# SamuelCancilla2/radar-point-cloud-tracking

Measured on AMD Instinct MI355X. Metric: Mpoints/s clustered+tracked, 1024-echo synthetic frames; 1/2/4/8-GPU scaling, higher is better.
Workload: dtype u8 echo / f32 geometry / f64 distance

## Files before the change

### radar-point-cloud-tracking_amd/csrc/stdbscan.hip

```cpp
#include <algorithm>
#include <cfloat>
#include <climits>
#include <cmath>
#include <cstdlib>
#include <cstring>
#include <mutex>
#include <type_traits>
#include <vector>

#include "common.h"
#include "dispatch.h"

#pragma clang fp contract(off)

namespace rpt {

namespace {

#include "stdbscan_shared.inc"
#include "stdbscan_grid.inc"
#include "stdbscan_core.inc"
#include "stdbscan_union.inc"
#include "stdbscan_label.inc"
#include "stdbscan_frames.inc"
// ... 17 lines not shown
  }
  double ms(int i) {
    float t = 0;
    (void)hipEventElapsedTime(&t, ev[i], ev[i + 1]);
    return t;
  }
  ~Timer() {
    for (auto& e : ev)
      if (e) (void)hipEventDestroy(e);
  }
};

}

struct DbscanState {
  Scratch arena;
  int dim = 2;
  int64_t n = 0;
  bool degenerate = false;
  int32_t min_samples = 0;
  Geom g{};
  int64_t C = 0, nt = 0;
  float4* pts = nullptr;
  int32_t *sorig = nullptr, *skey = nullptr, *cell_start = nullptr, *rep = nullptr;
  uint8_t *mutual = nullptr, *core = nullptr;
  float2* slab_t = nullptr;
  int32_t *parent = nullptr, *ccmin = nullptr, *cid = nullptr, *nc_list = nullptr;
  int32_t *occ = nullptr, *hpos = nullptr;
  const int32_t* n_occ_dev = nullptr;
  uint64_t* cell_min_pair = nullptr;
  bool cmin_ready = false;
  void* crec = nullptr;
  uint32_t* occ_bits = nullptr;
  uint4* pmask = nullptr;
  int union_cpw() const {
    if (ab().union_cpw) return ab().union_cpw;
    return n > (int64_t(1) << 24) ? 64 : 16;
  }
  uint32_t* min_bits = nullptr;
  int32_t* min_pref = nullptr;
  int64_t min_words() const { return n / 32 + 1; }
  int32_t* n_clusters_ptr() const { return min_pref + min_words(); }
  int32_t cluster_ids(hipStream_t st, int32_t* cell_key, int32_t* zero = nullptr);
  int32_t* cell_root = nullptr;
  bool bucket_allmin = false;
  bool k5_fused_path() const {
    return oct_ok() && ab().k5_mode == 0 && ab().k5_fused && !ab().k5_tiles;
  }
  int32_t* rowq = nullptr;
  int32_t* rowcnt = nullptr;
  bool rowq_ok = false;
  int tile_by = 0, tile_nbands = 0, tile_R = 0;
  bool use_label_tiles() const { return ab().k7_tiles && rowq_ok && dim == 2 && g.nz == 1; }
  unsigned tile_grid_blocks() const {
    return (unsigned)((((int64_t)g.nt * tile_nbands + 1) + 7) & ~(int64_t)7);
  }
  double slab_reach() const {
    return integral_t ? std::ceil(std::floor((double)g.epst) / g.ct)
                      : std::ceil((double)g.epst / g.ct) + 1.0;
  }
  bool oct_ok() const { return dim == 2 && g.nz == 1 && slab_reach() <= (double)kCwMaxR; }
  template <int D>
  const CellRec<D>* rec() const {
    return static_cast<const CellRec<D>*>(crec);
  }
  int32_t* slab = nullptr;
  bool spos_on = false;
  bool dense_slabs = false;
  int32_t* cell_min = nullptr;
  uint8_t* fok = nullptr;
  bool integral_t = false;
  bool all_mutual = false;
  bool cell_comp = false;
  bool cell_comp_ok() const {
    const AbSwitches& a = ab();
    return all_mutual && dim == 2 && a.union_list && a.union_pair && a.union_nm && a.cell_comp &&
           !use_label_tiles() && !a.uf_compress;
  }
  bool xy_points = false;
  bool may_xy = false;
  bool xy_rule() const {
    const AbSwitches& a = ab();
    return a.xy_points && dim == 2 && g.tfree && g.epst == std::floor(g.epst) && cell_comp_ok() &&
           k5_fused_path() && (int)slab_reach() <= 2 && a.k5_mask && !a.k7_tiles && a.k7_w == 32;
  }
  int32_t need_float4(const char* who) const {
    if (!xy_points) return RPT_OK;
    set_error("%s: internal: this state's sorted points are xy-only", who);
    return RPT_EHIP;
  }
  template <bool XY>
  Pt<XY>* points() const {
    return reinterpret_cast<Pt<XY>*>(pts);
  }
  int64_t* stmp = nullptr;
  Timer tm;

  template <int D>
  int32_t build_t(const float* x, const float* y, const float* z, int64_t stride, const float* t,
                  double eps_space, double eps_time, hipStream_t st);
  const void* given_bounds = nullptr;
  int32_t build(const float* x, const float* y, const float* z, int64_t stride, const float* t,
                int64_t n_, double eps_space, double eps_time, int32_t ms, bool timing,
                hipStream_t st);
  int32_t core_pass(hipStream_t st);
  int32_t union_pass(hipStream_t st, bool fused = false);
  int32_t labels_local(int32_t* labels, rpt_stdbscan_stats* stats, hipStream_t st);
  bool defer = false;
  int32_t fill_stats(int32_t n_clusters, rpt_stdbscan_stats* stats);
  int32_t labels_global(const int64_t* rep_orig, const int64_t* reps, int64_t nr,
                        int32_t* labels, hipStream_t st, const int64_t* nr_dev = nullptr);
// ... 90 lines not shown
    g.tfree = (g.rt >= 0 && ct == 1.0 && (double)g.rt <= std::floor((double)epst)) ? 1 : 0;
  }
  all_mutual = D == 2 && integral_t && ct == 1.0 && hb.n_finite_t == n && min_samples >= 1 &&
               epst >= 0.f && eps_space > 0.0 && 2.0 * cs * cs <= g.eps2 * (1.0 - 1e-6);
  C = g.cells;
  const int64_t C1 = C + 1;
  Budget bud;
  bud.add<Bounds>(1);
  for (int k = 0; k < 4; ++k) bud.add<uint32_t>(n);
  bud.add<int64_t>(radix_tmp_elems(n));
  bud.add<float4>(n);
  bud.add<int32_t>(n);
  bud.add<int32_t>(n);
  bud.add<int32_t>(C1 + 1);
  bud.add<int64_t>(scan_tmp_elems(C1 + 1) + scan_tmp_elems(n + 1));
  bud.add<uint8_t>(C1);
  bud.add<int32_t>(C1);
  bud.add<float2>(nt);
  bud.add<uint8_t>(n);
  bud.add<int32_t>(n);
  bud.add<int32_t>(n);
  bud.add<int32_t>(n + 1);
  bud.add<int32_t>(n + 1);
  bud.add<int32_t>(n);
  bud.add<uint8_t>(C1);
  bud.add<int32_t>(C1);
  bud.add<int32_t>(C1);
  bud.add<uint64_t>(C1);
  bud.add<uint32_t>(n / 32 + 1);
  bud.add<int32_t>(n / 32 + 2);
  bud.add<int32_t>(n + 1);
  bud.add<int32_t>(n + 1);
  bud.add<CellRec<D>>(C1);
  bud.add<uint32_t>(C1 / 32 + 2);
  bud.add<int32_t>(nt + 1);
  bud.add<int32_t>(nt + 1);
  bud.add<int32_t>(nt + 1);
  bud.add<int32_t>((size_t)(ny * nz * nt) + 1);
  bud.add<int32_t>((size_t)(ny * nz * nt) + 1);
  RPT_TRY(arena.reserve(bud.bytes, st));
  (void)arena.carve_n<Bounds>(1);
  uint32_t* keys = arena.carve_n<uint32_t>(n);
  uint32_t* vals = arena.carve_n<uint32_t>(n);
  uint32_t* keys_alt = arena.carve_n<uint32_t>(n);
  uint32_t* vals_alt = arena.carve_n<uint32_t>(n);
  pmask = reinterpret_cast<uint4*>(keys);
  int64_t* rtmp = arena.carve_n<int64_t>(radix_tmp_elems(n));
  pts = arena.carve_n<float4>(n);
  sorig = arena.carve_n<int32_t>(n);
  skey = arena.carve_n<int32_t>(n);
  cell_start = arena.carve_n<int32_t>(C1 + 1);
  stmp = arena.carve_n<int64_t>(scan_tmp_elems(C1 + 1) + scan_tmp_elems(n + 1));
  mutual = arena.carve_n<uint8_t>(C1);
  rep = arena.carve_n<int32_t>(C1);
  slab_t = arena.carve_n<float2>(nt);
  core = arena.carve_n<uint8_t>(n);
  parent = arena.carve_n<int32_t>(n);
  ccmin = arena.carve_n<int32_t>(n);
  cid = arena.carve_n<int32_t>(n + 1);
  nc_list = arena.carve_n<int32_t>(n + 1);
  slab = arena.carve_n<int32_t>(n);
  fok = arena.carve_n<uint8_t>(C1);
  cell_min = arena.carve_n<int32_t>(C1);
  cell_root = arena.carve_n<int32_t>(C1);
  cell_min_pair = arena.carve_n<uint64_t>(C1);
  min_bits = arena.carve_n<uint32_t>(n / 32 + 1);
  min_pref = arena.carve_n<int32_t>(n / 32 + 2);
  occ = arena.carve_n<int32_t>(n + 1);
  hpos = arena.carve_n<int32_t>(n + 1);
  CellRec<D>* cr = arena.carve_n<CellRec<D>>(C1);
  crec = cr;
  occ_bits = arena.carve_n<uint32_t>(C1 / 32 + 2);
  int32_t* slab_lo = arena.carve_n<int32_t>(nt + 1);
  int32_t* slab_occ = arena.carve_n<int32_t>(nt + 1);
  int32_t* occ_base = arena.carve_n<int32_t>(nt + 1);
  rowq = arena.carve_n<int32_t>((size_t)(ny * nz * nt) + 1);
  rowcnt = arena.carve_n<int32_t>((size_t)(ny * nz * nt) + 1);
  rowq_ok = false;
  if (!slab_lo || !rowcnt) {
    set_error("internal: scratch carve overflow");
    return RPT_ENOMEM;
  }
  bucket_allmin = false;
  const bool bucket = ab().k4_bucket && D == 2 && hb.n_finite_t == n && !hb.t_descends &&
                      (int64_t)nx * ny <= kBucketCells && nt < (int64_t(1) << 31);
  xy_points = may_xy && bucket && D == 2 && hb.n_finite_t == n && xy_rule();
  float2* const slab_t_w = xy_points ? slab_t : nullptr;
  if (bucket) {
    hipLaunchKernelGGL(k_slab_lo, dim3(grid_for(64 * (nt + 1), kBlock, 4096)), dim3(kBlock), 0,
                       st, t, n, g, slab_lo, occ_bits, (int64_t)(C1 / 32 + 2));
    const size_t hist_bytes = sizeof(int32_t) * (size_t)nx * ny;
    const int64_t avg = n / std::max<int64_t>(nt, 1);
    dense_slabs = avg > 8 * kChunkPts;
    spos_on = ab().label_orig == 2 || (ab().label_orig == 1 && dense_slabs);
    int32_t* spos_w = spos_on ? slab : nullptr;
    int64_t ch = avg > 8 * kChunkPts ? (avg + kChunkPts - 1) / kChunkPts : 1;
    ch = std::max<int64_t>(ch, (512 + nt - 1) / std::max<int64_t>(nt, 1));
    int CH = (int)std::min<int64_t>(ch, 64);
    while (CH > 1 && (int64_t)nt * CH * nx * ny > 4 * n) --CH;
    if (ab().slab_chunks > 0) CH = ab().slab_chunks;
    const bool coalesced_scan = CH >= 8 && (int64_t)nt * CH * nx * ny <= 4 * n &&
                                !ab().chunk_scan;
    if (CH > 1 && (int64_t)nt * CH * nx * ny <= 4 * n) {
      int32_t* hist_g = reinterpret_cast<int32_t*>(keys);
      RPT_HIP(hipFuncSetAttribute((const void*)k_slab_chunk_hist,
// ... 269 lines not shown
    hipLaunchKernelGGL(k_core_slow<3>, dim3(wave_grid(n)), dim3(kBlock), 0, st, pts, skey, g,
                       rec<3>(), occ_bits, slab_t, slow, n_slow, core);
  RPT_CHECK_LAUNCH();
  cmin_ready = cm != nullptr;
  tm.mark();
  return RPT_OK;
}

int32_t DbscanState::union_pass(hipStream_t st, bool fused) {
  cell_comp = false;
  if (degenerate) return RPT_OK;
  const AbSwitches& a = ab();
  const int uf_flags = a.uf_flags;
  const int gb = grid_for(n, kBlock, 2048);
  const int gw = wave_grid(n);
  const unsigned gp = (unsigned)((n + kBlock - 1) / kBlock);
  const int32_t* n_occ = n_occ_dev;
  auto* cmin = reinterpret_cast<unsigned long long*>(cell_min_pair);
  const bool listing = a.union_list && dim == 2;
  int32_t* plist = listing ? nc_list : nullptr;
  int32_t* pcount = listing ? nc_list + n : nullptr;
  const bool nm = dim == 2 && a.union_pair && a.union_nm;
  int32_t* nm_list = nm ? cid : nullptr;
  int32_t* nm_count = nm ? cid + n : nullptr;
  cell_comp = fused && cell_comp_ok();
  if (!cell_comp) RPT_TRY(need_float4("union_pass"));
  if (!cell_comp || !cmin_ready)
    hipLaunchKernelGGL(k_init_occ_cells, dim3(gb), dim3(kBlock), 0, st, occ, n_occ, C, rep,
                       cmin_ready ? nullptr : cmin, pcount, nm_count);
  if (!cmin_ready)
    hipLaunchKernelGGL(k_cell_min_pair, dim3(gb), dim3(kBlock), 0, st, skey, core, sorig, n, C,
                       cmin);
  if (cell_comp)
    hipLaunchKernelGGL(k_parent_init_cells, dim3(gb), dim3(kBlock), 0, st, occ, n_occ, C, cmin,
                       rep, parent, pcount, nm_count, min_bits, min_words(), cell_min);
  else
    hipLaunchKernelGGL(k_parent_init_pair, dim3(grid_for(n, kBlock * kPU, 2048)), dim3(kBlock), 0,
                       st, parent, n, core, skey, mutual, cmin, C, rep);
  int32_t* lstat_dev = nullptr;
  if (dim == 2) {
    uint4* pm = listing ? pmask : nullptr;
    if (a.union_pair)
      hipLaunchKernelGGL(k_union_cells_pair, dim3(gw), dim3(kBlock), 0, st, pts, g, occ, n_occ,
                         rec<2>(), occ_bits, slab_t, rep, mutual, sorig, parent, uf_flags, pm,
                         plist, pcount, union_cpw(), nm_list, nm_count);
    else
      hipLaunchKernelGGL((k_union_cells<2, false>), dim3(gw), dim3(kBlock), 0, st, pts, g,
                         cell_start, occ, n_occ, rec<2>(), occ_bits, slab_t, core, rep, mutual,
                         sorig, parent, uf_flags, pm, plist, pcount);
#ifdef RPT_AB
    if (listing && ab().stats) {
      static int32_t* buf = nullptr;
      if (!buf) (void)hipMalloc(&buf, 16);
      lstat_dev = buf;
      (void)hipMemsetAsync(lstat_dev, 0, 16, st);
    }
#endif
    if (listing) {
      const bool snap = ab().union_snap == 2 || (ab().union_snap == 1 && !dense_slabs);
      if (snap)
        hipLaunchKernelGGL(k_cell_root_snapshot, dim3(grid_for(n, kBlock, 4096)), dim3(kBlock),
                           0, st, occ, n_occ, rep, parent, g.cells, uf_flags, cell_root);
      const int32_t* croot = snap ? (const int32_t*)cell_root : nullptr;
      with_bool(xy_points, [&](auto xy) {
        hipLaunchKernelGGL(k_union_listed<xy.value>, dim3(gw), dim3(kBlock), 0, st,
                           points<xy.value>(), g, occ, rec<2>(), occ_bits, slab_t, core, rep,
                           mutual, sorig, parent, uf_flags, pm, plist, pcount, croot, lstat_dev);
      });
    }
    else
      hipLaunchKernelGGL((k_union_cells<2, true>), dim3(gw), dim3(kBlock), 0, st, pts, g,
                         cell_start, occ, n_occ, rec<2>(), occ_bits, slab_t, core, rep, mutual,
                         sorig, parent, uf_flags, pm, plist, pcount);
    if (cell_comp) {
    } else if (nm)
      hipLaunchKernelGGL(k_union_nm<2>, dim3(gw), dim3(kBlock), 0, st, pts, g, cell_start,
                         rec<2>(), slab_t, core, rep, mutual, sorig, parent, nm_list, nm_count);
    else
// ... 42 lines not shown
                       occ, n_occ_dev, C, mutual, rep, cell_root, zero, min_bits, W, cell_key);
  } else {
    RPT_HIP(hipMemsetAsync(min_bits, 0, sizeof(uint32_t) * W, st));
    if (zero) RPT_HIP(hipMemsetAsync(zero, 0, sizeof(int32_t), st));
    if (cell_key)
      hipLaunchKernelGGL(k_fill_i32, dim3(grid_for(C, kBlock, 8192)), dim3(kBlock), 0, st,
                         cell_key, C, INT_MAX);
  }
  hipLaunchKernelGGL(k_ccmin, dim3(tile_grid(n)), dim3(kBlock), 0, st, parent, core, n, sorig,
                     ccmin, min_bits, nc_list, nc_list + n, skey, mutual,
                     cr ? (const int32_t*)cell_root : nullptr, C, cell_key);
  hipLaunchKernelGGL(k_word_popc, dim3(grid_for(W, kBlock, 2048)), dim3(kBlock), 0, st, min_bits,
                     W, min_pref);
  RPT_CHECK_LAUNCH();
  return exclusive_scan_total_i32(min_pref, min_pref, W, st);
}

int32_t DbscanState::labels_local(int32_t* labels, rpt_stdbscan_stats* stats, hipStream_t st) {
  const int gb = grid_for(n, kBlock, 2048);
  if (degenerate) {
    hipLaunchKernelGGL(k_isolated_labels, dim3(gb), dim3(kBlock), 0, st, labels, n,
                       min_samples <= 0 ? 1 : 0);
    RPT_CHECK_LAUNCH();
    if (stats) {
      stats->n_points = n;
      stats->n_core = min_samples <= 0 ? n : 0;
      stats->n_clusters = min_samples <= 0 ? (int32_t)n : 0;
    }
    return RPT_OK;
  }
  int32_t* nc_count = nc_list + n;
  const MinRank mr{min_bits, min_pref};
  const unsigned glc = (unsigned)((grid_for(n, kBlock * kPU, 2048) + 7) & ~7);
  if (cell_comp) {
    const int64_t W = min_words();
    hipLaunchKernelGGL(k_cell_comp, dim3(grid_for(n, kBlock, 2048)), dim3(kBlock), 0, st, parent,
                       occ, n_occ_dev, C, rep, sorig, cell_min, min_bits, nc_count);
    hipLaunchKernelGGL(k_word_popc, dim3(grid_for(W, kBlock, 2048)), dim3(kBlock), 0, st,
                       min_bits, W, min_pref);
    RPT_CHECK_LAUNCH();
    RPT_TRY(exclusive_scan_total_i32(min_pref, min_pref, W, st));
    with_bool(spos_on, [&](auto orig) {
      hipLaunchKernelGGL(k_label_core_cells<orig.value>, dim3(glc), dim3(kBlock), 0, st, skey,
                         core, orig.value ? slab : sorig, n, C, cell_min, mr, labels, nc_list,
                         nc_count, cid + n, n_clusters_ptr());
    });
  } else {
    RPT_TRY(cluster_ids(st, cell_min, nc_count));
    if (spos_on)
      hipLaunchKernelGGL(k_label_core_orig, dim3(glc), dim3(kBlock), 0, st, ccmin, n, slab, mr,
                         labels);
    else
      hipLaunchKernelGGL(k_label_core, dim3(glc), dim3(kBlock), 0, st, ccmin, n, sorig, mr,
                         labels);
  }
  if (!cell_comp || ab().k7_w != 32 || use_label_tiles()) RPT_TRY(need_float4("labels_local"));
  int32_t* kstat = nullptr;
#ifdef RPT_AB
  if (ab().stats) {
    static int32_t* buf = nullptr;
    if (!buf) (void)hipMalloc(&buf, 16);
    kstat = buf;
    (void)hipMemsetAsync(kstat, 0, 16, st);
  }
#endif
#ifdef RPT_AB
  if (use_label_tiles())
    hipLaunchKernelGGL((k_label_tiles<false>), dim3(tile_grid_blocks()), dim3(kTileBlock), 0, st,
                       g, tile_R, tile_by, tile_nbands, (int64_t)g.nt * tile_nbands, occ,
                       n_occ_dev, rowq, rec<2>(), mutual, occ_bits, slab_t, pts, ccmin, cell_min,
                       sorig, mr, min_samples, labels);
  else if (cell_comp && ab().k7_w == 64)
    hipLaunchKernelGGL((k_label<2, false, 64, true>), dim3(wave_grid(n)), dim3(kBlock), 0, st,
                       pts, skey, g, rec<2>(), occ_bits, slab_t, (const int32_t*)nullptr,
                       cell_min, mutual, sorig, mr, nc_list, nc_count, labels,
                       (int32_t*)nullptr, core);
  else if (dim == 2 && ab().k7_w == 64)
    hipLaunchKernelGGL((k_label<2, false, 64>), dim3(wave_grid(n)), dim3(kBlock), 0, st, pts,
                       skey, g, rec<2>(), occ_bits, slab_t, ccmin, cell_min, mutual, sorig, mr,
                       nc_list, nc_count, labels);
  else
#endif
  if (cell_comp && xy_points)
    hipLaunchKernelGGL((k_label<2, false, 32, true, true>), dim3(wave_grid(n)), dim3(kBlock), 0,
                       st, reinterpret_cast<const Pt<true>*>(pts), skey, g, rec<2>(), occ_bits,
                       slab_t, (const int32_t*)nullptr, cell_min, mutual, sorig, mr, nc_list,
                       nc_count, labels, kstat, core);
  else if (cell_comp)
    hipLaunchKernelGGL((k_label<2, false, 32, true>), dim3(wave_grid(n)), dim3(kBlock), 0, st,
                       pts, skey, g, rec<2>(), occ_bits, slab_t, (const int32_t*)nullptr,
                       cell_min, mutual, sorig, mr, nc_list, nc_count, labels, kstat, core);
  else if (dim == 2)
    hipLaunchKernelGGL((k_label<2, false, 32>),
                       dim3(wave_grid(n)), dim3(kBlock), 0, st, pts, skey, g,
                       rec<2>(), occ_bits, slab_t, ccmin, cell_min, mutual, sorig, mr, nc_list,
                       nc_count, labels, kstat);
  else
    hipLaunchKernelGGL((k_label<3, false, 64>),
                       dim3(wave_grid(n)), dim3(kBlock), 0, st, pts, skey, g,
                       rec<3>(), occ_bits, slab_t, ccmin, cell_min, mutual, sorig, mr, nc_list,
                       nc_count, labels);
  RPT_CHECK_LAUNCH();
#ifdef RPT_AB
  if (kstat) {
    int32_t ks[4] = {0, 0, 0, 0};
    (void)hipMemcpyAsync(ks, kstat, 16, hipMemcpyDeviceToHost, st);
    (void)hipStreamSynchronize(st);
    std::fprintf(stderr,
                 "[rpt stats] n=%lld label: queued=%d core_in_window=%d searched=%d labelled=%d\n",
                 (long long)n, ks[0], ks[1], ks[2], ks[3]);
  }
#endif
  tm.mark();
  if (stats && defer) return RPT_OK;
  if (stats) {
    int32_t ncl = 0;
    RPT_HIP(hipMemcpyAsync(&ncl, n_clusters_ptr(), sizeof(int32_t), hipMemcpyDeviceToHost, st));
    RPT_TRY(wait_stream(st));
    RPT_TRY(fill_stats(ncl, stats));
  }
  return RPT_OK;
}

int32_t DbscanState::fill_stats(int32_t ncl, rpt_stdbscan_stats* stats) {
// ... 447 lines not shown
```

### radar-point-cloud-tracking_amd/csrc/stdbscan_label.inc

```

__global__ __launch_bounds__(kBlock) void k_fill_i32(int32_t* p, int64_t n, int32_t v) {
  for (int64_t i = (int64_t)blockIdx.x * blockDim.x + threadIdx.x; i < n;
       i += (int64_t)gridDim.x * blockDim.x)
    p[i] = v;
}

struct MinRank {
  const uint32_t* bits;
  const int32_t* pref;
  __device__ __forceinline__ int32_t operator[](int32_t m) const {
    const uint32_t w = bits[m >> 5];
    return pref[m >> 5] + __popc(w & ((1u << (m & 31)) - 1u));
  }
};

__global__ void k_word_popc(const uint32_t* __restrict__ bits, int64_t words,
                            int32_t* __restrict__ out) {
  for (int64_t i = (int64_t)blockIdx.x * blockDim.x + threadIdx.x; i < words;
       i += (int64_t)gridDim.x * blockDim.x)
    out[i] = __popc(bits[i]);
}

__global__ __launch_bounds__(kBlock) void k_cell_roots(int32_t* parent,
                                                      const int32_t* __restrict__ occ,
// ... 177 lines not shown
#pragma unroll
    for (int u = 0; u < kPU; ++u) {
      const int64_t i = tile + (int64_t)u * kBlock + threadIdx.x;
      if (i < n && own[u] >= 0)
        labels[i] = pr[u] + __popc(w[u] & ((1u << (own[u] & 31)) - 1u));
    }
  }
}

__global__ __launch_bounds__(kBlock) void k_cell_comp(int32_t* parent,
                                                     const int32_t* __restrict__ occ,
                                                     const int32_t* __restrict__ n_occ,
                                                     int64_t cells,
                                                     const int32_t* __restrict__ rep,
                                                     const int32_t* __restrict__ sorig,
                                                     int32_t* __restrict__ cell_key,
                                                     uint32_t* __restrict__ min_bits,
                                                     int32_t* __restrict__ zero) {
  if (blockIdx.x == 0 && threadIdx.x == 0) *zero = 0;
  const int64_t m = *n_occ;
  for (int64_t q = (int64_t)blockIdx.x * blockDim.x + threadIdx.x; q < m;
       q += (int64_t)gridDim.x * blockDim.x) {
    const int32_t c = occ[q];
    if ((int64_t)c >= cells) continue;
    const int r = rep[c];
    if (r < 0) continue;
    const int root = uf_find(parent, r);
    const int32_t k = sorig[root];
    cell_key[c] = k;
    if (root == r) atomicOr(min_bits + (k >> 5), 1u << (k & 31));
  }
}

struct AppendSpos {
  const int32_t* spos;
  __device__ int32_t operator()(int64_t i) const { return spos[i]; }
};
template <bool ORIG>
__global__ __launch_bounds__(kBlock) void k_label_core_cells(
    const int32_t* __restrict__ skey, const uint8_t* __restrict__ core,
    const int32_t* __restrict__ perm, int64_t n, int64_t cells,
    const int32_t* __restrict__ cell_key, MinRank cid, int32_t* __restrict__ labels,
    int32_t* __restrict__ nc_list, int32_t* __restrict__ nc_count,
    const int32_t* __restrict__ guard, int32_t* __restrict__ n_clusters) {
  if (blockIdx.x == 0 && threadIdx.x == 0 && *guard != 0) *n_clusters = -1;
  const int64_t T = (n + (int64_t)kBlock * kPU - 1) / ((int64_t)kBlock * kPU);
  const bool xm = (gridDim.x & 7) == 0;
  const int64_t xg = blockIdx.x & 7, nbx = gridDim.x >> 3;
  const int64_t t_lo = xm ? T * xg / 8 : blockIdx.x, t_hi = xm ? T * (xg + 1) / 8 : T;
  const int64_t t_step = xm ? nbx : gridDim.x;
  for (int64_t ti = t_lo + (xm ? (int64_t)(blockIdx.x >> 3) : 0); ti < t_hi; ti += t_step) {
    const int64_t tile = ti * kBlock * kPU;
    int32_t pv[kPU], k[kPU];
    uint32_t c[kPU];
    if (ORIG) {
#pragma unroll
      for (int u = 0; u < kPU; ++u)
        pv[u] = __builtin_nontemporal_load(perm + min(tile + (int64_t)u * kBlock + threadIdx.x,
                                                       n - 1));
#pragma unroll
      for (int u = 0; u < kPU; ++u) {
        k[u] = skey[pv[u]];
        c[u] = core[pv[u]];
      }
    } else {
#pragma unroll
      for (int u = 0; u < kPU; ++u) {
        const int64_t s = min(tile + (int64_t)u * kBlock + threadIdx.x, n - 1);
        k[u] = skey[s];
        c[u] = core[s];
        pv[u] = perm[s];
      }
    }
    int32_t own[kPU];
    uint32_t inb = 0, cb = 0;
#pragma unroll
    for (int u = 0; u < kPU; ++u) {
      const bool in = tile + (int64_t)u * kBlock + threadIdx.x < n;
      const bool q = in && c[u] != 0u && k[u] >= 0 && (int64_t)k[u] < cells;
      inb |= in ? (1u << u) : 0u;
      cb |= (in && c[u] != 0u) ? (1u << u) : 0u;
      const int32_t v = cell_key[q ? k[u] : 0];
      own[u] = (q && v != INT_MAX) ? v : -1;
    }
    uint32_t w[kPU];
    int32_t pr[kPU];
#pragma unroll
    for (int u = 0; u < kPU; ++u) {
      const int32_t m = own[u] >= 0 ? own[u] : 0;
      w[u] = cid.bits[m >> 5];
      pr[u] = cid.pref[m >> 5];
    }
#pragma unroll
    for (int u = 0; u < kPU; ++u) {
      if (own[u] >= 0) {
        const int32_t lab = pr[u] + __popc(w[u] & ((1u << (own[u] & 31)) - 1u));
        if (ORIG)
          labels[tile + (int64_t)u * kBlock + threadIdx.x] = lab;
        else
          labels[pv[u]] = lab;
      }
    }
    if (ORIG)
      block_append_bits(tile, inb & ~cb, nc_list, nc_count, AppendSpos{perm});
    else
      block_append_bits(tile, inb & ~cb, nc_list, nc_count);
  }
}

template <int D, bool GLOBAL, int W = 64, bool ALLMUT = false, bool XY = false>
__global__ __launch_bounds__(kBlock, 6) void k_label(const Pt<XY>* __restrict__ pts,
                                                 const int32_t* __restrict__ skey, Geom g,
                                                 const CellRec<D>* __restrict__ crec,
                                                 const uint32_t* __restrict__ occ_bits,
                                                 const float2* __restrict__ slab_t,
                                                 const int32_t* __restrict__ key_of,
                                                 const int32_t* __restrict__ cell_key,
                                                 const uint8_t* __restrict__ mutual,
                                                 const int32_t* __restrict__ sorig,
                                                 MinRank cid,
                                                 const int32_t* __restrict__ nc_list,
                                                 const int32_t* __restrict__ nc_count,
                                                 int32_t* __restrict__ labels,
                                                 int32_t* __restrict__ kstat = nullptr,
                                                 const uint8_t* __restrict__ core_of = nullptr) {
  static_assert(!ALLMUT || (D == 2 && !GLOBAL), "all-mutual grids are 2-D, local runs");
  static_assert(!XY || ALLMUT, "xy points only on all-mutual grids");
  static_assert(W == 32 || W == 64, "a point per wave or per half-wave");
  constexpr int P = 64 / W;
  const int lane = threadIdx.x & 63;
  const int hl = lane & (W - 1);
  const int h0 = lane - hl;
  const int shift = (W == 64) ? 0 : h0;
  auto gbal = [&](bool v) -> uint64_t {
    const uint64_t b = __ballot(v);
    return (W == 64) ? b : ((b >> shift) & 0xffffffffull);
  };
  auto gmin = [&](int v) -> int {
    v = row_reduce<16>(v, OpMin{});
    v = min(v, __shfl_xor(v, 16));
    if (W == 64) v = min(v, __shfl_xor(v, 32));
    return v;
  };
  const int64_t nc = *nc_count;
  const XcdRange xr = xcd_items((nc + P - 1) / P, true);
  for (int64_t qp = xr.first; qp < xr.end; qp += xr.step) {
    const int64_t q = qp * P + (lane / W);
    if (q >= nc) continue;
    const int s = nc_list[q];
    const int32_t key = skey[s];
    int best = INT_MAX;
#ifdef RPT_AB
    bool st_core = false, st_search = false;
#endif
    if ((int64_t)key < g.cells) {
      const float4 p = load_pt<XY>(pts, s);
      int cx, cy, cz;
      decode_key<D>(key, g, cx, cy, cz);
      const Window w = XY ? slab_window<D>(cx, cy, cz, g.slab_of_key(key), g)
                          : make_window<D, false>(cx, cy, cz, p.w, p.w, g, slab_t);
      for (int base = 0; base < w.total; base += W * kR) {
        int64_t c[kR];
        int ck[kR], cb[kR], ce[kR], cls[kR], mu[kR];
#pragma unroll
        for (int k = 0; k < kR; ++k) {
          const int qq = base + k * W + hl;
          c[k] = (qq < w.total) ? window_cell<D>(w, qq, g, slab_t, p.w, p.w) : -1;
        }
#pragma unroll
        for (int k = 0; k < kR; ++k) ck[k] = (c[k] >= 0) ? cell_key[c[k]] : INT_MAX;
        int v = INT_MAX;
#pragma unroll
        for (int k = 0; k < kR; ++k) {
          cb[k] = ce[k] = cls[k] = mu[k] = 0;
          if (ck[k] != INT_MAX) {
            const CellRec<D> cr = crec[c[k]];
            cb[k] = cr.b;
            ce[k] = cr.e;
            mu[k] = ALLMUT ? 1 : mutual[c[k]];
            cls[k] = classify<D, XY>(p, rec_boxA<D>(cr), rec_boxB(cr), g);
            if (cls[k] == 1) v = min(v, ck[k]);
          }
        }
        best = min(best, gmin(v));
#ifdef RPT_AB
        {
          bool anyc = false;
#pragma unroll
          for (int k = 0; k < kR; ++k) anyc = anyc || ck[k] != INT_MAX;
          st_core = st_core || gbal(anyc) != 0;
        }
#endif
        uint32_t pend = 0;
#pragma unroll
        for (int k = 0; k < kR; ++k) pend |= (cls[k] == 2) ? (1u << k) : 0u;
        while (true) {
          int mine = INT_MAX, mk = -1;
#pragma unroll
          for (int k = 0; k < kR; ++k)
            if (((pend >> k) & 1u) && ck[k] < best && ck[k] < mine) {
              mine = ck[k];
              mk = k;
            }
          const int mm = gmin(mine);
          if (mm == INT_MAX) break;
#ifdef RPT_AB
          st_search = true;
#endif
          const uint64_t at = gbal(mine == mm);
          const int l = h0 + __ffsll((unsigned long long)at) - 1;
          const int kl = __shfl(mk, l);
          int bsel = 0, esel = 0, msel = 0;
#pragma unroll
          for (int k = 0; k < kR; ++k)
            if (k == kl) {
              bsel = cb[k];
              esel = ce[k];
              msel = mu[k];
            }
          if (lane == l) pend &= ~(1u << kl);
          const int bl = __shfl(bsel, l), el = __shfl(esel, l);
          if (ALLMUT || __shfl(msel, l)) {
            bool hit = false;
            for (int j0 = bl; j0 < el && !hit; j0 += 2 * W) {
              const int j = j0 + hl, j2 = j + W;
              const bool v1 = j < el, v2 = j2 < el;
              int k1, k2;
              if (ALLMUT) {
                k1 = (v1 && core_of[j]) ? 0 : -1;
                k2 = (v2 && core_of[j2]) ? 0 : -1;
              } else {
                k1 = v1 ? key_of[j] : -1;
                k2 = v2 ? key_of[j2] : -1;
              }
              const float4 p1 = v1 ? load_pt<XY>(pts, j) : p;
              const float4 p2 = v2 ? load_pt<XY>(pts, j2) : p;
              hit = gbal((k1 >= 0 && adjacent<D, XY>(p, p1, g)) ||
                         (k2 >= 0 && adjacent<D, XY>(p, p2, g))) != 0;
            }
            if (hit) best = mm;
          } else {
            int lb = INT_MAX;
            for (int j0 = bl; j0 < el; j0 += 2 * W) {
              const int j = j0 + hl, j2 = j + W;
              const bool v1 = j < el, v2 = j2 < el;
              const int m1 = v1 ? key_of[j] : -1, m2 = v2 ? key_of[j2] : -1;
              const float4 p1 = v1 ? load_pt<XY>(pts, j) : p;
              const float4 p2 = v2 ? load_pt<XY>(pts, j2) : p;
              if (m1 >= 0 && m1 < best && m1 < lb && adjacent<D, XY>(p, p1, g)) lb = m1;
              if (m2 >= 0 && m2 < best && m2 < lb && adjacent<D, XY>(p, p2, g)) lb = m2;
            }
            best = min(best, gmin(lb));
          }
        }
      }
    }
    if (hl == 0) {
      int32_t out = -1;
      if (best != INT_MAX) out = GLOBAL ? best : cid[best];
      labels[sorig[s]] = out;
#ifdef RPT_AB
      if (kstat) {
        atomicAdd(&kstat[0], 1);
        if (st_core) atomicAdd(&kstat[1], 1);
        if (st_search) atomicAdd(&kstat[2], 1);
        if (best != INT_MAX) atomicAdd(&kstat[3], 1);
      }
#endif
    }
  }
}

#ifdef RPT_AB
#include "stdbscan_ab.inc"
#endif

__global__ __launch_bounds__(kBlock) void k_isolated_labels(int32_t* labels, int64_t n,
                                                           int singletons) {
  for (int64_t i = (int64_t)blockIdx.x * blockDim.x + threadIdx.x; i < n;
       i += (int64_t)gridDim.x * blockDim.x)
    labels[i] = singletons ? (int32_t)i : -1;
}


__global__ void k_core_to_orig(const uint8_t* __restrict__ core, const int32_t* __restrict__ sorig,
                               int64_t n, uint8_t* __restrict__ out) {
  for (int64_t s = (int64_t)blockIdx.x * blockDim.x + threadIdx.x; s < n;
       s += (int64_t)gridDim.x * blockDim.x)
// ... 169 lines not shown
```

### radar-point-cloud-tracking_amd/csrc/stdbscan_union.inc

```

__global__ __launch_bounds__(kBlock) void k_cell_min_pair(const int32_t* __restrict__ skey,
                                                         const uint8_t* __restrict__ core,
                                                         const int32_t* __restrict__ sorig,
                                                         int64_t n, int64_t cells,
                                                         unsigned long long* __restrict__ cmin) {
  const int lane = threadIdx.x & 63;
  for (int64_t s0 = (int64_t)blockIdx.x * blockDim.x; s0 < n;
       s0 += (int64_t)gridDim.x * blockDim.x) {
    const int64_t s = s0 + threadIdx.x;
    const int key = (s < n) ? skey[s] : -1;
    uint64_t v = (s < n && core[s] && (int64_t)key < cells)
                     ? (((uint64_t)(uint32_t)sorig[s] << 32) | (uint32_t)s)
                     : ~0ull;
#pragma unroll
    for (int off = 1; off < 64; off <<= 1) {
      const uint32_t olo = (uint32_t)__shfl_up((int)(uint32_t)v, off, 64);
      const uint32_t ohi = (uint32_t)__shfl_up((int)(uint32_t)(v >> 32), off, 64);
      const int ok = __shfl_up(key, off, 64);
      if (lane >= off && ok == key) v = min(v, ((uint64_t)ohi << 32) | olo);
    }
    const int next = __shfl_down(key, 1, 64);
    if ((lane == 63 || next != key) && key >= 0 && v != ~0ull)
      atomicMin(cmin + key, (unsigned long long)v);
  }
// ... 30 lines not shown
  for (int64_t tile = (int64_t)blockIdx.x * kBlock * kPU; tile < n;
       tile += (int64_t)gridDim.x * kBlock * kPU) {
    int32_t k[kPU];
    uint32_t c[kPU];
#pragma unroll
    for (int u = 0; u < kPU; ++u) {
      const int64_t s = min(tile + (int64_t)u * kBlock + threadIdx.x, n - 1);
      k[u] = skey[s];
      c[u] = core[s];
    }
    bool q[kPU];
    unsigned long long m[kPU];
    uint32_t mu[kPU];
#pragma unroll
    for (int u = 0; u < kPU; ++u) {
      q[u] = c[u] != 0u && k[u] >= 0 && (int64_t)k[u] < cells;
      const int32_t kk = q[u] ? k[u] : 0;
      m[u] = cmin[kk];
      mu[u] = mutual[kk];
    }
#pragma unroll
    for (int u = 0; u < kPU; ++u) {
      const int64_t s = tile + (int64_t)u * kBlock + threadIdx.x;
      if (s < n) {
        const int32_t r = (int32_t)(uint32_t)m[u];
        if (q[u] && r == (int32_t)s) rep[k[u]] = r;
        parent[s] = (q[u] && mu[u]) ? r : (int32_t)s;
      }
    }
  }
}

__global__ __launch_bounds__(kBlock) void k_parent_init_cells(
    const int32_t* __restrict__ occ, const int32_t* __restrict__ n_occ, int64_t cells,
    const unsigned long long* __restrict__ cmin, int32_t* __restrict__ rep,
    int32_t* __restrict__ parent, int32_t* __restrict__ zero_counter,
    int32_t* __restrict__ zero_counter2, uint32_t* __restrict__ zwords, int64_t nzw,
    int32_t* __restrict__ cell_key) {
  if (blockIdx.x == 0 && threadIdx.x == 0) {
    if (zero_counter) *zero_counter = 0;
    if (zero_counter2) *zero_counter2 = 0;
  }
  const int64_t t0 = (int64_t)blockIdx.x * blockDim.x + threadIdx.x;
  const int64_t ts = (int64_t)gridDim.x * blockDim.x;
  for (int64_t i = t0; i < nzw; i += ts) zwords[i] = 0u;
  for (int64_t i = t0; i < cells; i += ts) cell_key[i] = INT_MAX;
  const int64_t m = *n_occ;
  for (int64_t q = t0; q < m; q += ts) {
    const int32_t c = occ[q];
    if ((int64_t)c >= cells) continue;
    const unsigned long long v = cmin[c];
    const int32_t r = (v != ~0ull) ? (int32_t)(uint32_t)v : -1;
    rep[c] = r;
    if (r >= 0) parent[r] = r;
  }
}

__device__ __forceinline__ int uf_load(const int32_t* p) {
  return __hip_atomic_load(p, __ATOMIC_RELAXED, __HIP_MEMORY_SCOPE_AGENT);
}
__device__ __forceinline__ void uf_store(int32_t* p, int v) {
  __hip_atomic_store(p, v, __ATOMIC_RELAXED, __HIP_MEMORY_SCOPE_AGENT);
}
__device__ __forceinline__ int uf_find(int32_t* parent, int x, bool halve = true) {
  while (true) {
    const int p = uf_load(parent + x);
    if (p == x) return x;
    const int gp = uf_load(parent + p);
    if (gp == p) return p;
    if (halve) uf_store(parent + x, gp);
    x = gp;
  }
}
__device__ __forceinline__ void uf_unite(int32_t* parent, const int32_t* __restrict__ sorig,
                                         int a, int b, bool halve = true) {
  while (true) {
    a = uf_find(parent, a, halve);
    b = uf_find(parent, b, halve);
    if (a == b) return;
    if (sorig[a] < sorig[b]) {
      const int tmp = a;
      a = b;
      b = tmp;
    }
    const int old = atomicCAS(parent + a, a, b);
    if (old == a) return;
    a = old;
// ... 196 lines not shown
    if (lane == 0) base = atomicAdd(&n, c);
    base = __shfl(base, 0);
    const bool fits = base + c <= Cap;
    if (fits) {
      if (lane == 0) atomicMax(&valid, base + c);
    } else {
      if (lane == 0) base = atomicAdd(gcount, c);
      base = __shfl(base, 0);
    }
    if ((m >> lane) & 1ull) {
      const int at = base + __popcll(m & ((1ull << lane) - 1ull));
      if (fits)
        buf[at] = v;
      else
        glist[at] = v;
    }
  }
  __device__ void flush(int lane, int32_t* glist, int32_t* gcount) {
    const int cnt = valid;
    int base = 0;
    if (lane == 0 && cnt) base = atomicAdd(gcount, cnt);
    base = __shfl(base, 0);
    for (int k = lane; k < cnt; k += 64) glist[base + k] = buf[k];
  }
};
__device__ __forceinline__ bool block_last_wave(int* done, int lane) {
  __threadfence_block();
  int last = 0;
  if (lane == 0) last = atomicAdd(done, 1) == (int)(blockDim.x / 64) - 1;
  last = __shfl(last, 0);
  if (last) __threadfence_block();
  return last != 0;
}
__global__ __launch_bounds__(kBlock, 6) void k_union_cells_pair(
    const float4* __restrict__ pts, Geom g, const int32_t* __restrict__ occ,
    const int32_t* __restrict__ n_occ, const CellRec<2>* __restrict__ crec,
    const uint32_t* __restrict__ occ_bits, const float2* __restrict__ slab_t,
    const int32_t* __restrict__ rep, const uint8_t* __restrict__ mutual,
    const int32_t* __restrict__ sorig, int32_t* __restrict__ parent, int uf_flags,
    uint4* __restrict__ pmask, int32_t* __restrict__ plist, int32_t* __restrict__ pcount,
    int cpw, int32_t* __restrict__ nm_list, int32_t* __restrict__ nm_count) {
  constexpr int W = 32;
  const int lane = threadIdx.x & 63;
  const int hl = lane & (W - 1), h0 = lane - hl;
  auto hbal = [&](bool v) -> uint32_t { return (uint32_t)(__ballot(v) >> h0); };
  const bool halve = !(uf_flags & 1);
  const int64_t no = *n_occ;
  const int64_t items = (no + cpw - 1) / cpw;
  const XcdRange xr = xcd_items(items, (uf_flags & 2) != 0);
  __shared__ BlockList<1024> s_pl;
  __shared__ BlockList<256> s_nm;
  __shared__ int s_done;
  if (threadIdx.x == 0) {
    s_pl.init();
    s_nm.init();
    s_done = 0;
  }
  __syncthreads();
  for (int64_t it = xr.first; it < xr.end; it += xr.step) {
    int ql = -1, cal = INT_MAX, ral = -1;
    uint8_t mal = 0;
    if (lane < cpw && it * cpw + lane < no) ql = (int)(it * cpw + lane);
    if (ql >= 0) cal = occ[ql];
    if ((int64_t)cal < g.cells) {
      ral = rep[cal];
      mal = mutual[cal];
// ... 18 lines not shown
      ra_rec.b = __shfl(rl.b, lsrc);
      ra_rec.e = __shfl(rl.e, lsrc);
      ra_rec.x0 = __shfl(rl.x0, lsrc);
      ra_rec.x1 = __shfl(rl.x1, lsrc);
      ra_rec.y0 = __shfl(rl.y0, lsrc);
      ra_rec.y1 = __shfl(rl.y1, lsrc);
      ra_rec.t0 = __shfl(rl.t0, lsrc);
      ra_rec.t1 = __shfl(rl.t1, lsrc);
      if (lq >= 0) {
        const float4 A1 = rec_boxA<2>(ra_rec), A2 = rec_boxB(ra_rec);
        int cx, cy, cz;
        decode_key<2>(ca, g, cx, cy, cz);
        const int sa = g.slab_of_key(ca);
        const Window w = make_window<2, false>(cx, cy, cz, A2.z, A2.w, g, slab_t, sa);
        for (int base = 0; base < w.total; base += W * kR) {
          int64_t cb[kR];
          uint32_t wb[kR];
          int rb[kR], cls[kR];
#pragma unroll
          for (int k = 0; k < kR; ++k) {
            const int qq = base + k * W + hl;
            cb[k] = (qq < w.total) ? window_cell<2>(w, qq, g, slab_t, A2.z, A2.w) : -1;
            if (cb[k] <= (int64_t)ca) cb[k] = -1;
          }
#pragma unroll
          for (int k = 0; k < kR; ++k) wb[k] = (cb[k] >= 0) ? occ_bits[cb[k] >> 5] : 0u;
#pragma unroll
          for (int k = 0; k < kR; ++k) {
            rb[k] = -1;
            cls[k] = 0;
            if (cb[k] >= 0 && ((wb[k] >> (cb[k] & 31)) & 1u)) {
              const CellRec<2> cr = crec[cb[k]];
              const int r = rep[cb[k]];
              const uint8_t m = mutual[cb[k]];
              if (r >= 0 && m) {
                rb[k] = r;
                cls[k] = classify_cells<2>(A1, rec_boxA<2>(cr), A2, rec_boxB(cr), g);
              }
            }
          }
          if (pmask && base == 0) {
            uint32_t wd[kR];
#pragma unroll
            for (int k = 0; k < kR; ++k) wd[k] = hbal(cls[k] == 2);
            static_assert(kR == 4, "the 128-bit pmask holds 4 x 32 window positions");
            if (hl == 0)
              pmask[q] = (w.total < 128)
                             ? make_uint4(wd[0], wd[1], wd[2], wd[3] & ~kPmaskFull)
                             : make_uint4(0u, 0u, 0u, kPmaskFull);
            any_und = w.total >= 128 || (wd[0] | wd[1] | wd[2] | wd[3]) != 0u;
          }
          const int rA = uf_find(parent, ra, halve);
#pragma unroll
          for (int k = 0; k < kR; ++k) {
            const int rt = (cls[k] == 1) ? uf_find(parent, rb[k], halve) : -1;
            bool pend = rt >= 0 && rt != rA;
            bool mine = false;
            uint32_t pm = hbal(pend);
            while (pm) {
              const int l = h0 + __ffs(pm) - 1;
              const int v = __shfl(rt, l);
              mine = mine || (lane == l);
              pend = pend && (rt != v);
              pm = hbal(pend);
            }
            if (mine) uf_unite(parent, sorig, rA, rt, halve);
          }
// ... 250 lines not shown
```

Measured before the change: 9079.

## Add per-cell core bitmaps to prune union and label neighbor scans

Builds a core_bits bitmap marking cells with a core representative while parent init runs. Parent init now walks all cells densely instead of the occupied list. The union pass reads this bitmap instead of occ_bits and skips the mutual load. The label kernel enumerates only set bits in the 5-wide window rows using ballots and nth-set-bit selection, and a new near_bits dilation lets non-core points with no core cell nearby be labeled noise directly, skipping the noise list. The cost is extra kernels, more index arithmetic, and dense cell iteration in parent init.

```diff
diff --git a/radar-point-cloud-tracking_amd/csrc/stdbscan.hip b/radar-point-cloud-tracking_amd/csrc/stdbscan.hip
--- a/radar-point-cloud-tracking_amd/csrc/stdbscan.hip
+++ b/radar-point-cloud-tracking_amd/csrc/stdbscan.hip
@@ -73,6 +73,7 @@
   bool cmin_ready = false;
   void* crec = nullptr;
   uint32_t* occ_bits = nullptr;
+  uint32_t *core_bits = nullptr, *near_bits = nullptr;
   uint4* pmask = nullptr;
   int union_cpw() const {
     if (ab().union_cpw) return ab().union_cpw;
@@ -118,6 +119,8 @@
     return all_mutual && dim == 2 && a.union_list && a.union_pair && a.union_nm && a.cell_comp &&
            !use_label_tiles() && !a.uf_compress;
   }
+  bool core_bits_ok() const { return cell_comp_ok() && g.rt >= 0; }
+  bool near_bits_ok() const { return core_bits_ok() && !dense_slabs; }
   bool xy_points = false;
   bool may_xy = false;
   bool xy_rule() const {
@@ -274,6 +277,8 @@
   bud.add<int32_t>(n + 1);
   bud.add<int32_t>(n + 1);
   bud.add<CellRec<D>>(C1);
+  bud.add<uint32_t>(C1 / 32 + 2);
+  bud.add<uint32_t>(C1 / 32 + 2);
   bud.add<uint32_t>(C1 / 32 + 2);
   bud.add<int32_t>(nt + 1);
   bud.add<int32_t>(nt + 1);
@@ -313,6 +318,8 @@
   CellRec<D>* cr = arena.carve_n<CellRec<D>>(C1);
   crec = cr;
   occ_bits = arena.carve_n<uint32_t>(C1 / 32 + 2);
+  core_bits = arena.carve_n<uint32_t>(C1 / 32 + 2);
+  near_bits = arena.carve_n<uint32_t>(C1 / 32 + 2);
   int32_t* slab_lo = arena.carve_n<int32_t>(nt + 1);
   int32_t* slab_occ = arena.carve_n<int32_t>(nt + 1);
   int32_t* occ_base = arena.carve_n<int32_t>(nt + 1);
@@ -648,18 +655,24 @@
     hipLaunchKernelGGL(k_cell_min_pair, dim3(gb), dim3(kBlock), 0, st, skey, core, sorig, n, C,
                        cmin);
   if (cell_comp)
-    hipLaunchKernelGGL(k_parent_init_cells, dim3(gb), dim3(kBlock), 0, st, occ, n_occ, C, cmin,
-                       rep, parent, pcount, nm_count, min_bits, min_words(), cell_min);
+    hipLaunchKernelGGL(k_parent_init_cells, dim3(gb), dim3(kBlock), 0, st, C, cmin, rep, parent,
+                       pcount, nm_count, min_bits, min_words(),
+                       near_bits_ok() ? (int32_t*)nullptr : cell_min, occ_bits, core_bits,
+                       (int64_t)((C + 1) / 32 + 2));
   else
     hipLaunchKernelGGL(k_parent_init_pair, dim3(grid_for(n, kBlock * kPU, 2048)), dim3(kBlock), 0,
                        st, parent, n, core, skey, mutual, cmin, C, rep);
   int32_t* lstat_dev = nullptr;
   if (dim == 2) {
     uint4* pm = listing ? pmask : nullptr;
-    if (a.union_pair)
-      hipLaunchKernelGGL(k_union_cells_pair, dim3(gw), dim3(kBlock), 0, st, pts, g, occ, n_occ,
-                         rec<2>(), occ_bits, slab_t, rep, mutual, sorig, parent, uf_flags, pm,
-                         plist, pcount, union_cpw(), nm_list, nm_count);
+    if (a.union_pair && cell_comp)
+      hipLaunchKernelGGL(k_union_cells_pair<true>, dim3(gw), dim3(kBlock), 0, st, pts, g, occ,
+                         n_occ, rec<2>(), core_bits, slab_t, rep, mutual, sorig, parent, uf_flags,
+                         pm, plist, pcount, union_cpw(), nm_list, nm_count);
+    else if (a.union_pair)
+      hipLaunchKernelGGL(k_union_cells_pair<false>, dim3(gw), dim3(kBlock), 0, st, pts, g, occ,
+                         n_occ, rec<2>(), occ_bits, slab_t, rep, mutual, sorig, parent, uf_flags,
+                         pm, plist, pcount, union_cpw(), nm_list, nm_count);
     else
       hipLaunchKernelGGL((k_union_cells<2, false>), dim3(gw), dim3(kBlock), 0, st, pts, g,
                          cell_start, occ, n_occ, rec<2>(), occ_bits, slab_t, core, rep, mutual,
@@ -768,8 +781,15 @@
   int32_t* nc_count = nc_list + n;
   const MinRank mr{min_bits, min_pref};
   const unsigned glc = (unsigned)((grid_for(n, kBlock * kPU, 2048) + 7) & ~7);
+  const bool bits = cell_comp && core_bits_ok();
+  const bool nearb = cell_comp && near_bits_ok();
   if (cell_comp) {
     const int64_t W = min_words();
+    if (nearb) {
+      const int nbw = (int)((C + 1) / 32 + 2);
+      hipLaunchKernelGGL(k_near_bits, dim3(grid_for(nbw, kBlock, 2048)), dim3(kBlock), 0, st,
+                         core_bits, nbw, g.nx, g.ny, g.rt, near_bits);
+    }
     hipLaunchKernelGGL(k_cell_comp, dim3(grid_for(n, kBlock, 2048)), dim3(kBlock), 0, st, parent,
                        occ, n_occ_dev, C, rep, sorig, cell_min, min_bits, nc_count);
     hipLaunchKernelGGL(k_word_popc, dim3(grid_for(W, kBlock, 2048)), dim3(kBlock), 0, st,
@@ -777,9 +797,12 @@
     RPT_CHECK_LAUNCH();
     RPT_TRY(exclusive_scan_total_i32(min_pref, min_pref, W, st));
     with_bool(spos_on, [&](auto orig) {
-      hipLaunchKernelGGL(k_label_core_cells<orig.value>, dim3(glc), dim3(kBlock), 0, st, skey,
-                         core, orig.value ? slab : sorig, n, C, cell_min, mr, labels, nc_list,
-                         nc_count, cid + n, n_clusters_ptr());
+      with_bool(nearb, [&](auto nr) {
+        hipLaunchKernelGGL((k_label_core_cells<orig.value, nr.value>), dim3(glc), dim3(kBlock), 0,
+                           st, skey, core, orig.value ? slab : sorig, n, C, cell_min, mr, labels,
+                           nc_list, nc_count, cid + n, n_clusters_ptr(),
+                           nr.value ? (const uint32_t*)near_bits : nullptr);
+      });
     });
   } else {
     RPT_TRY(cluster_ids(st, cell_min, nc_count));
@@ -807,10 +830,12 @@
                        n_occ_dev, rowq, rec<2>(), mutual, occ_bits, slab_t, pts, ccmin, cell_min,
                        sorig, mr, min_samples, labels);
   else if (cell_comp && ab().k7_w == 64)
-    hipLaunchKernelGGL((k_label<2, false, 64, true>), dim3(wave_grid(n)), dim3(kBlock), 0, st,
-                       pts, skey, g, rec<2>(), occ_bits, slab_t, (const int32_t*)nullptr,
-                       cell_min, mutual, sorig, mr, nc_list, nc_count, labels,
-                       (int32_t*)nullptr, core);
+    with_bool(bits, [&](auto b) {
+      hipLaunchKernelGGL((k_label<2, false, 64, true, false, b.value>), dim3(wave_grid(n)),
+                         dim3(kBlock), 0, st, pts, skey, g, rec<2>(), occ_bits, slab_t,
+                         (const int32_t*)nullptr, cell_min, mutual, sorig, mr, nc_list, nc_count,
+                         labels, (int32_t*)nullptr, core, core_bits);
+    });
   else if (dim == 2 && ab().k7_w == 64)
     hipLaunchKernelGGL((k_label<2, false, 64>), dim3(wave_grid(n)), dim3(kBlock), 0, st, pts,
                        skey, g, rec<2>(), occ_bits, slab_t, ccmin, cell_min, mutual, sorig, mr,
@@ -818,14 +843,17 @@
   else
 #endif
   if (cell_comp && xy_points)
-    hipLaunchKernelGGL((k_label<2, false, 32, true, true>), dim3(wave_grid(n)), dim3(kBlock), 0,
-                       st, reinterpret_cast<const Pt<true>*>(pts), skey, g, rec<2>(), occ_bits,
-                       slab_t, (const int32_t*)nullptr, cell_min, mutual, sorig, mr, nc_list,
-                       nc_count, labels, kstat, core);
+    hipLaunchKernelGGL((k_label<2, false, 32, true, true, true>), dim3(wave_grid(n)),
+                       dim3(kBlock), 0, st, reinterpret_cast<const Pt<true>*>(pts), skey, g,
+                       rec<2>(), occ_bits, slab_t, (const int32_t*)nullptr, cell_min, mutual,
+                       sorig, mr, nc_list, nc_count, labels, kstat, core, core_bits);
   else if (cell_comp)
-    hipLaunchKernelGGL((k_label<2, false, 32, true>), dim3(wave_grid(n)), dim3(kBlock), 0, st,
-                       pts, skey, g, rec<2>(), occ_bits, slab_t, (const int32_t*)nullptr,
-                       cell_min, mutual, sorig, mr, nc_list, nc_count, labels, kstat, core);
+    with_bool(bits, [&](auto b) {
+      hipLaunchKernelGGL((k_label<2, false, 32, true, false, b.value>), dim3(wave_grid(n)),
+                         dim3(kBlock), 0, st, pts, skey, g, rec<2>(), occ_bits, slab_t,
+                         (const int32_t*)nullptr, cell_min, mutual, sorig, mr, nc_list, nc_count,
+                         labels, kstat, core, core_bits);
+    });
   else if (dim == 2)
     hipLaunchKernelGGL((k_label<2, false, 32>),
                        dim3(wave_grid(n)), dim3(kBlock), 0, st, pts, skey, g,
diff --git a/radar-point-cloud-tracking_amd/csrc/stdbscan_label.inc b/radar-point-cloud-tracking_amd/csrc/stdbscan_label.inc
--- a/radar-point-cloud-tracking_amd/csrc/stdbscan_label.inc
+++ b/radar-point-cloud-tracking_amd/csrc/stdbscan_label.inc
@@ -233,17 +233,42 @@
   }
 }
 
+__global__ __launch_bounds__(kBlock) void k_near_bits(const uint32_t* __restrict__ core_bits,
+                                                     int nbw, int nx, int ny, int rt,
+                                                     uint32_t* __restrict__ near_bits) {
+  auto word = [&](int k) -> uint32_t {
+    const uint32_t v = core_bits[min(max(k, 0), nbw - 1)];
+    return (k >= 0 && k < nbw) ? v : 0u;
+  };
+  for (int w = blockIdx.x * blockDim.x + threadIdx.x; w < nbw; w += gridDim.x * blockDim.x) {
+    uint32_t acc = 0;
+    for (int ds = -rt; ds <= rt; ++ds) {
+#pragma unroll
+      for (int dy = -2; dy <= 2; ++dy) {
+        const int64_t p = (int64_t)w * 32 + ((int64_t)ds * ny + dy) * nx - 2;
+        const int k = (int)(p >> 5), sh = (int)(p & 31);
+        const uint32_t a = word(k), b = word(k + 1), c = word(k + 2);
+        uint64_t x = (((uint64_t)b << 32) | a) >> sh;
+        x |= sh ? ((uint64_t)c << (64 - sh)) : 0ull;
+        acc |= (uint32_t)(x | (x >> 1) | (x >> 2) | (x >> 3) | (x >> 4));
+      }
+    }
+    near_bits[w] = acc;
+  }
+}
+
 struct AppendSpos {
   const int32_t* spos;
   __device__ int32_t operator()(int64_t i) const { return spos[i]; }
 };
-template <bool ORIG>
+template <bool ORIG, bool NEAR>
 __global__ __launch_bounds__(kBlock) void k_label_core_cells(
     const int32_t* __restrict__ skey, const uint8_t* __restrict__ core,
     const int32_t* __restrict__ perm, int64_t n, int64_t cells,
     const int32_t* __restrict__ cell_key, MinRank cid, int32_t* __restrict__ labels,
     int32_t* __restrict__ nc_list, int32_t* __restrict__ nc_count,
-    const int32_t* __restrict__ guard, int32_t* __restrict__ n_clusters) {
+    const int32_t* __restrict__ guard, int32_t* __restrict__ n_clusters,
+    const uint32_t* __restrict__ near) {
   if (blockIdx.x == 0 && threadIdx.x == 0 && *guard != 0) *n_clusters = -1;
   const int64_t T = (n + (int64_t)kBlock * kPU - 1) / ((int64_t)kBlock * kPU);
   const bool xm = (gridDim.x & 7) == 0;
@@ -274,7 +299,14 @@
       }
     }
     int32_t own[kPU];
-    uint32_t inb = 0, cb = 0;
+    uint32_t inb = 0, cb = 0, far = 0;
+    uint32_t nw[kPU];
+#pragma unroll
+    for (int u = 0; u < kPU; ++u) {
+      const bool in = tile + (int64_t)u * kBlock + threadIdx.x < n;
+      nw[u] = ~0u;
+      if (NEAR && in && c[u] == 0u && k[u] >= 0 && (int64_t)k[u] < cells) nw[u] = near[k[u] >> 5];
+    }
 #pragma unroll
     for (int u = 0; u < kPU; ++u) {
       const bool in = tile + (int64_t)u * kBlock + threadIdx.x < n;
@@ -284,6 +316,10 @@
       const int32_t v = cell_key[q ? k[u] : 0];
       own[u] = (q && v != INT_MAX) ? v : -1;
     }
+    if (NEAR) {
+#pragma unroll
+      for (int u = 0; u < kPU; ++u) far |= ((nw[u] >> (k[u] & 31)) & 1u) ? 0u : (1u << u);
+    }
     uint32_t w[kPU];
     int32_t pr[kPU];
 #pragma unroll
@@ -300,16 +336,35 @@
           labels[tile + (int64_t)u * kBlock + threadIdx.x] = lab;
         else
           labels[pv[u]] = lab;
+      } else if ((far >> u) & 1u) {
+        if (ORIG)
+          labels[tile + (int64_t)u * kBlock + threadIdx.x] = -1;
+        else
+          labels[pv[u]] = -1;
       }
     }
     if (ORIG)
-      block_append_bits(tile, inb & ~cb, nc_list, nc_count, AppendSpos{perm});
+      block_append_bits(tile, inb & ~cb & ~far, nc_list, nc_count, AppendSpos{perm});
     else
-      block_append_bits(tile, inb & ~cb, nc_list, nc_count);
-  }
-}
-
-template <int D, bool GLOBAL, int W = 64, bool ALLMUT = false, bool XY = false>
+      block_append_bits(tile, inb & ~cb & ~far, nc_list, nc_count);
+  }
+}
+
+__device__ __forceinline__ int nth_set_bit(uint64_t m, int n) {
+  int pos = 0;
+#pragma unroll
+  for (int s = 32; s > 0; s >>= 1) {
+    const int c = __popcll(m & ((1ull << s) - 1ull));
+    if (n >= c) {
+      n -= c;
+      m >>= s;
+      pos += s;
+    }
+  }
+  return pos;
+}
+
+template <int D, bool GLOBAL, int W = 64, bool ALLMUT = false, bool XY = false, bool BITS = false>
 __global__ __launch_bounds__(kBlock, 6) void k_label(const Pt<XY>* __restrict__ pts,
                                                  const int32_t* __restrict__ skey, Geom g,
                                                  const CellRec<D>* __restrict__ crec,
@@ -324,8 +379,10 @@
                                                  const int32_t* __restrict__ nc_count,
                                                  int32_t* __restrict__ labels,
                                                  int32_t* __restrict__ kstat = nullptr,
-                                                 const uint8_t* __restrict__ core_of = nullptr) {
+                                                 const uint8_t* __restrict__ core_of = nullptr,
+                                                 const uint32_t* __restrict__ core_bits = nullptr) {
   static_assert(!ALLMUT || (D == 2 && !GLOBAL), "all-mutual grids are 2-D, local runs");
+  static_assert(!BITS || ALLMUT, "core_bits is built on the per-cell path of all-mutual grids");
   static_assert(!XY || ALLMUT, "xy points only on all-mutual grids");
   static_assert(W == 32 || W == 64, "a point per wave or per half-wave");
   constexpr int P = 64 / W;
@@ -360,19 +417,63 @@
       decode_key<D>(key, g, cx, cy, cz);
       const Window w = XY ? slab_window<D>(cx, cy, cz, g.slab_of_key(key), g)
                           : make_window<D, false>(cx, cy, cz, p.w, p.w, g, slab_t);
-      for (int base = 0; base < w.total; base += W * kR) {
-        int64_t c[kR];
-        int ck[kR], cb[kR], ce[kR], cls[kR], mu[kR];
-#pragma unroll
-        for (int k = 0; k < kR; ++k) {
-          const int qq = base + k * W + hl;
-          c[k] = (qq < w.total) ? window_cell<D>(w, qq, g, slab_t, p.w, p.w) : -1;
+      constexpr int NK = BITS ? 1 : kR;
+      const int nrows = BITS ? 5 * w.nS : 1;
+      for (int rbase = 0; rbase < nrows; rbase += W) {
+      uint64_t bx[5] = {0, 0, 0, 0, 0};
+      int tot = w.total;
+      if (BITS) {
+        const int row = rbase + hl;
+        const int ss = row / 5, yy = row - ss * 5;
+        const int y = w.y0 + yy;
+        uint32_t f = 0;
+        if (row < nrows && y >= 0 && y < g.ny) {
+          const int xlo = max(w.x0, 0), xhi = min(w.x0 + 4, g.nx - 1);
+          const int64_t pb = ((int64_t)(w.s0 + ss) * g.ny + y) * g.nx + xlo;
+          const uint64_t two = ((uint64_t)core_bits[(pb >> 5) + 1] << 32) | core_bits[pb >> 5];
+          f = ((uint32_t)(two >> (pb & 31)) & ((1u << (xhi - xlo + 1)) - 1u)) << (xlo - w.x0);
         }
-#pragma unroll
-        for (int k = 0; k < kR; ++k) ck[k] = (c[k] >= 0) ? cell_key[c[k]] : INT_MAX;
+        tot = 0;
+#pragma unroll
+        for (int xx = 0; xx < 5; ++xx) {
+          bx[xx] = gbal((f >> xx) & 1u);
+          tot += __popcll(bx[xx]);
+        }
+      }
+      for (int base = 0; base < tot; base += W * NK) {
+        int64_t c[NK];
+        int ck[NK], cb[NK], ce[NK], cls[NK], mu[NK];
+        if (BITS) {
+          int idx = base + hl, qq = -1;
+          if (idx < tot) {
+            uint64_t m = 0;
+            int xs = 0;
+            bool found = false;
+#pragma unroll
+            for (int xx = 0; xx < 5; ++xx) {
+              const int cn = __popcll(bx[xx]);
+              if (!found && idx < cn) {
+                m = bx[xx];
+                xs = xx;
+                found = true;
+              }
+              if (!found) idx -= cn;
+            }
+            qq = (rbase + nth_set_bit(m, idx)) * 5 + xs;
+          }
+          c[0] = (qq >= 0) ? window_cell<D>(w, qq, g, slab_t, p.w, p.w) : -1;
+        } else {
+#pragma unroll
+          for (int k = 0; k < NK; ++k) {
+            const int qq = base + k * W + hl;
+            c[k] = (qq < w.total) ? window_cell<D>(w, qq, g, slab_t, p.w, p.w) : -1;
+          }
+        }
+#pragma unroll
+        for (int k = 0; k < NK; ++k) ck[k] = (c[k] >= 0) ? cell_key[c[k]] : INT_MAX;
         int v = INT_MAX;
 #pragma unroll
-        for (int k = 0; k < kR; ++k) {
+        for (int k = 0; k < NK; ++k) {
           cb[k] = ce[k] = cls[k] = mu[k] = 0;
           if (ck[k] != INT_MAX) {
             const CellRec<D> cr = crec[c[k]];
@@ -388,17 +489,17 @@
         {
           bool anyc = false;
 #pragma unroll
-          for (int k = 0; k < kR; ++k) anyc = anyc || ck[k] != INT_MAX;
+          for (int k = 0; k < NK; ++k) anyc = anyc || ck[k] != INT_MAX;
           st_core = st_core || gbal(anyc) != 0;
         }
 #endif
         uint32_t pend = 0;
 #pragma unroll
-        for (int k = 0; k < kR; ++k) pend |= (cls[k] == 2) ? (1u << k) : 0u;
+        for (int k = 0; k < NK; ++k) pend |= (cls[k] == 2) ? (1u << k) : 0u;
         while (true) {
           int mine = INT_MAX, mk = -1;
 #pragma unroll
-          for (int k = 0; k < kR; ++k)
+          for (int k = 0; k < NK; ++k)
             if (((pend >> k) & 1u) && ck[k] < best && ck[k] < mine) {
               mine = ck[k];
               mk = k;
@@ -413,7 +514,7 @@
           const int kl = __shfl(mk, l);
           int bsel = 0, esel = 0, msel = 0;
 #pragma unroll
-          for (int k = 0; k < kR; ++k)
+          for (int k = 0; k < NK; ++k)
             if (k == kl) {
               bsel = cb[k];
               esel = ce[k];
@@ -455,6 +556,7 @@
           }
         }
       }
+      }
     }
     if (hl == 0) {
       int32_t out = -1;
diff --git a/radar-point-cloud-tracking_amd/csrc/stdbscan_union.inc b/radar-point-cloud-tracking_amd/csrc/stdbscan_union.inc
--- a/radar-point-cloud-tracking_amd/csrc/stdbscan_union.inc
+++ b/radar-point-cloud-tracking_amd/csrc/stdbscan_union.inc
@@ -86,11 +86,11 @@
 }
 
 __global__ __launch_bounds__(kBlock) void k_parent_init_cells(
-    const int32_t* __restrict__ occ, const int32_t* __restrict__ n_occ, int64_t cells,
-    const unsigned long long* __restrict__ cmin, int32_t* __restrict__ rep,
+    int64_t cells, const unsigned long long* __restrict__ cmin, int32_t* __restrict__ rep,
     int32_t* __restrict__ parent, int32_t* __restrict__ zero_counter,
     int32_t* __restrict__ zero_counter2, uint32_t* __restrict__ zwords, int64_t nzw,
-    int32_t* __restrict__ cell_key) {
+    int32_t* __restrict__ cell_key, const uint32_t* __restrict__ occ_bits,
+    uint32_t* __restrict__ core_bits, int64_t nbw) {
   if (blockIdx.x == 0 && threadIdx.x == 0) {
     if (zero_counter) *zero_counter = 0;
     if (zero_counter2) *zero_counter2 = 0;
@@ -98,15 +98,22 @@
   const int64_t t0 = (int64_t)blockIdx.x * blockDim.x + threadIdx.x;
   const int64_t ts = (int64_t)gridDim.x * blockDim.x;
   for (int64_t i = t0; i < nzw; i += ts) zwords[i] = 0u;
-  for (int64_t i = t0; i < cells; i += ts) cell_key[i] = INT_MAX;
-  const int64_t m = *n_occ;
-  for (int64_t q = t0; q < m; q += ts) {
-    const int32_t c = occ[q];
-    if ((int64_t)c >= cells) continue;
-    const unsigned long long v = cmin[c];
-    const int32_t r = (v != ~0ull) ? (int32_t)(uint32_t)v : -1;
-    rep[c] = r;
-    if (r >= 0) parent[r] = r;
+  const int lane = threadIdx.x & 63;
+  for (int64_t i = t0; i - lane < nbw * 32; i += ts) {
+    const bool in = i < cells;
+    const bool o = in && ((occ_bits[i >> 5] >> (i & 31)) & 1u);
+    int32_t r = -1;
+    if (o) {
+      const unsigned long long v = cmin[i];
+      r = (v != ~0ull) ? (int32_t)(uint32_t)v : -1;
+      rep[i] = r;
+      if (r >= 0) parent[r] = r;
+    }
+    const uint64_t b = __ballot(r >= 0);
+    const int64_t w = (i - lane) >> 5;
+    if (lane == 0) core_bits[w] = (uint32_t)b;
+    if (lane == 32 && w + 1 < nbw) core_bits[w + 1] = (uint32_t)(b >> 32);
+    if (cell_key && in) cell_key[i] = INT_MAX;
   }
 }
 
@@ -369,6 +376,7 @@
   if (last) __threadfence_block();
   return last != 0;
 }
+template <bool CORE>
 __global__ __launch_bounds__(kBlock, 6) void k_union_cells_pair(
     const float4* __restrict__ pts, Geom g, const int32_t* __restrict__ occ,
     const int32_t* __restrict__ n_occ, const CellRec<2>* __restrict__ crec,
@@ -453,7 +461,7 @@
             if (cb[k] >= 0 && ((wb[k] >> (cb[k] & 31)) & 1u)) {
               const CellRec<2> cr = crec[cb[k]];
               const int r = rep[cb[k]];
-              const uint8_t m = mutual[cb[k]];
+              const uint8_t m = CORE ? (uint8_t)1 : mutual[cb[k]];
               if (r >= 0 && m) {
                 rb[k] = r;
                 cls[k] = classify_cells<2>(A1, rec_boxA<2>(cr), A2, rec_boxB(cr), g);
```

Result: faster. 9312, median of 6 (+2.6%).
